# kcat/openal-soft

Measured on NVIDIA H100. Metric: voice-samples/s mixed (HRTF, bsinc24, 1024-frame updates), higher is better.
Workload: dtype f32

## Files before the change

### openal-soft_b200/csrc/async_ptx.cuh

```cuda
#pragma once
#include <cstdint>
#include <cuda_runtime.h>

namespace b200mix {

__device__ __forceinline__ uint32_t smem_u32(const void *p)
{ return static_cast<uint32_t>(__cvta_generic_to_shared(p)); }

__device__ __forceinline__ void mbar_init(uint64_t *bar, uint32_t count)
{ asm volatile("mbarrier.init.shared::cta.b64 [%0], %1;" :: "r"(smem_u32(bar)), "r"(count) : "memory"); }
__device__ __forceinline__ void mbar_fence_init()
{ asm volatile("fence.mbarrier_init.release.cluster;" ::: "memory"); }
__device__ __forceinline__ void mbar_expect_tx(uint64_t *bar, uint32_t bytes)
{ asm volatile("mbarrier.arrive.expect_tx.shared::cta.b64 _, [%0], %1;" :: "r"(smem_u32(bar)), "r"(bytes) : "memory"); }
__device__ __forceinline__ void mbar_arrive(uint64_t *bar)
{ asm volatile("mbarrier.arrive.shared::cta.b64 _, [%0];" :: "r"(smem_u32(bar)) : "memory"); }
__device__ __forceinline__ bool mbar_try_wait(uint64_t *bar, uint32_t parity)
{
    uint32_t ok;
    asm volatile("{\n\t.reg .pred p;\n\t"
                 "mbarrier.try_wait.parity.shared::cta.b64 p, [%1], %2;\n\t"
                 "selp.u32 %0, 1, 0, p;\n\t}"
                 : "=r"(ok) : "r"(smem_u32(bar)), "r"(parity) : "memory");
    return ok != 0u;
}
__device__ __forceinline__ void mbar_wait(uint64_t *bar, uint32_t parity)
{ while(!mbar_try_wait(bar, parity)) { } }

__device__ __forceinline__ void bulk_g2s(void *dst_smem, const void *src_gmem, uint32_t bytes, uint64_t *bar)
{
    asm volatile("cp.async.bulk.shared::cluster.global.mbarrier::complete_tx::bytes [%0], [%1], %2, [%3];"
        :: "r"(smem_u32(dst_smem)), "l"(src_gmem), "r"(bytes), "r"(smem_u32(bar)) : "memory");
}
__device__ __forceinline__ void fence_proxy_async_smem()
{ asm volatile("fence.proxy.async.shared::cta;" ::: "memory"); }

__device__ __forceinline__ void griddep_wait() { asm volatile("griddepcontrol.wait;" ::: "memory"); }
__device__ __forceinline__ void griddep_launch_dependents()
{ asm volatile("griddepcontrol.launch_dependents;" ::: "memory"); }

__device__ __forceinline__ uint64_t wgmma_smem_desc(uint32_t saddr, uint32_t lbo_bytes, uint32_t sbo_bytes)
{
    return uint64_t((saddr >> 4) & 0x3fffu) | (uint64_t((lbo_bytes >> 4) & 0x3fffu) << 16)
        | (uint64_t((sbo_bytes >> 4) & 0x3fffu) << 32);
}
__device__ __forceinline__ void wgmma_fence() { asm volatile("wgmma.fence.sync.aligned;" ::: "memory"); }
__device__ __forceinline__ void wgmma_commit() { asm volatile("wgmma.commit_group.sync.aligned;" ::: "memory"); }
template<int N> __device__ __forceinline__ void wgmma_wait()
{ asm volatile("wgmma.wait_group.sync.aligned %0;" :: "n"(N) : "memory"); }
__device__ __forceinline__ void wgmma_m64n16k8_tf32(float (&d)[8], uint64_t adesc, uint64_t bdesc, bool accumulate)
{
    asm volatile("{\n\t.reg .pred p;\n\tsetp.ne.b32 p, %10, 0;\n\t"
                 "wgmma.mma_async.sync.aligned.m64n16k8.f32.tf32.tf32 "
                 "{%0,%1,%2,%3,%4,%5,%6,%7}, %8, %9, p, 1, 1;\n\t}"
        : "+f"(d[0]), "+f"(d[1]), "+f"(d[2]), "+f"(d[3]), "+f"(d[4]), "+f"(d[5]), "+f"(d[6]), "+f"(d[7])
        : "l"(adesc), "l"(bdesc), "r"(uint32_t(accumulate)) : "memory");
}

}
```

### openal-soft_b200/csrc/mixer_kernels.cuh

```cuda
#pragma once
#include <cstddef>
#include <cstdint>
#include <cuda_runtime.h>

#include "voice_structs.hpp"
#include "async_ptx.cuh"

namespace b200mix {

constexpr int kLine = 1024;
constexpr int kHrirLen = 128;
constexpr int kHist = 64;
constexpr int kEdge = 24;
constexpr int kPad = 48;
constexpr int kResBuf = kLine + 256 + kPad;
constexpr int kSrcSizeMax = kResBuf - kEdge;
constexpr int kAccumLen = kLine + kHrirLen;
constexpr float kSilence = 0.00001f;
constexpr float kEps = 1.1920929e-07f;

constexpr uint32_t kVfStatic = 1u<<2, kVfLooping = 1u<<3, kVfHrtf = 1u<<4;
constexpr uint32_t kVfFading = 1u<<8, kVfHaveBuffer = 1u<<9, kVfCoefDirty = 1u<<10;
constexpr uint32_t kUpNoBuffer = 1u<<11;
constexpr uint32_t kVfChannelMask = 0xffu<<16;
// ... 810 lines not shown
            }
        }
        if(t == 0)
            newGain[c] = early ? (cg + step*float(fadeLen)) : tg;
    }
}

__device__ __forceinline__ void store_dry_gains(float *cur, const float *newGain, uint32_t cd, int t)
{
    if(t == 0)
        for(uint32_t c = 0;c < cd;++c) cur[c] = newGain[c];
}

__device__ __forceinline__ void write_back_voice(const MixParams &P, VoiceRec &rec, uint32_t v,
    uint4 h1, uint32_t flags, uint32_t vstate, uint32_t increment, bool haveBuffer, bool isQueue,
    uint4 qh, const uint32_t *qitems, bool looping, uint32_t loopStart, uint32_t loopEnd,
    uint32_t bufFrames)
{
    uint32_t newFlags = (flags | kVfFading) & ~kVfCoefDirty;
    uint32_t newState = vstate;
    uint32_t buffersDone = 0u;
    int32_t pos = int32_t(h1.x); uint32_t frac = h1.y;
    if(vstate == 2u) newState = 0u;
    else
    {
        frac += increment*P.frames;
        const uint32_t done = frac >> 16;
        pos = add_sat(pos, int32_t(done));
        frac &= 0xffffu;
        if(haveBuffer && pos > 0 && isQueue)
        {
            uint32_t item = qh.x ? qh.y : kNoLoop;
            while(item != kNoLoop)
            {
                const uint32_t len = P.buffers[qitems[item]].frames;
                if(len > uint32_t(pos)) break;
                pos -= int32_t(len);
                ++buffersDone;
                item = (item + 1u < qh.x) ? item + 1u : qh.z;
            }
            if(item == kNoLoop) { newFlags &= ~kVfHaveBuffer; newState = 2u; }
            else if(item != qh.y) P.qhdr[v].y = item;
        }
        else if(haveBuffer && pos > 0)
        {
            if(looping)
            {
                uint32_t up = uint32_t(pos);
                if(up >= loopEnd)
                    pos = int32_t((up-loopStart)%(loopEnd-loopStart) + loopStart);
            }
            else if(uint32_t(pos) >= bufFrames)
            {
                newFlags &= ~kVfHaveBuffer;
                newState = 2u;
            }
        }
        if(!haveBuffer) newState = 2u;
        rec.pos = pos; rec.frac = frac;
    }
    rec.flags = newFlags;
    rec.state = newState;
    if(P.results)
        P.results[v] = VoiceResult{pos, frac,
            newState == 1u ? 1u : (newState == 2u ? 2u : (1u<<7)), buffersDone};
}

template<int GS, int GROUPS, int CDR>
__device__ __forceinline__ void store_partial_row(const float (&accD)[CDR][kLine/GS], unsigned char *smem,
    float *partial, int g, int t)
{
    constexpr int SPT = kLine / GS;
    const size_t row = blockIdx.x;
    __syncthreads();
    float *stage = reinterpret_cast<float*>(smem);
    float *pd = partial + row*(size_t(CDR)*kLine);
    if(GROUPS == 1)
    {
        #pragma unroll
        for(int c = 0;c < CDR;++c)
            #pragma unroll
            for(int r = 0;r < SPT;++r)
                pd[c*kLine + t + r*GS] = accD[c][r];
    }
    else
    {
        for(int gg = 0;gg < GROUPS;++gg)
        {
            if(g == gg)
            {
                #pragma unroll
                for(int c = 0;c < CDR;++c)
                    #pragma unroll
                    for(int r = 0;r < SPT;++r)
                    {
                        float *dst = stage + c*kLine + t + r*GS;
                        if(gg == 0) *dst = accD[c][r]; else *dst += accD[c][r];
                    }
            }
            __syncthreads();
        }
        for(int o = threadIdx.x;o < CDR*kLine;o += GS*GROUPS) pd[o] = stage[o];
    }
}

constexpr int kMixGS = 64, kMixGroups = 2;

template<int GS, int GROUPS, int CDR>
__global__ void __launch_bounds__(GS*GROUPS, GS*GROUPS != 128 ? 1 : (CDR == 0 ? 5 : 3))
k_mix_voices(const MixParams P)
{
    using Smem = GroupSmem<CDR>;
    static_assert(CDR == 0 || sizeof(Smem)*GROUPS >= size_t(CDR)*kLine*sizeof(float),
        "the partial row is staged in the groups' storage");
    extern __shared__ __align__(16) unsigned char smem_raw[];
    const int g = threadIdx.x / GS;
    const int t = threadIdx.x % GS;
    Smem &S = reinterpret_cast<Smem*>(smem_raw)[g];
    const int bar = 1 + g;
    constexpr int SPT = kLine / GS;

    float accD[CDR > 0 ? CDR : 1][SPT];
    #pragma unroll
    for(int c = 0;c < (CDR > 0 ? CDR : 1);++c)
        #pragma unroll
        for(int r = 0;r < SPT;++r) accD[c][r] = 0.0f;

    const uint32_t n = P.frames;
    if(t == 0) { mbar_init(&S.tmaBar, 1u); mbar_fence_init(); }
    uint32_t tmaPhase = 0u;
    group_sync(bar, GS);

    const uint32_t groups = gridDim.x*GROUPS;
    for(uint32_t oi = CDR > 0 ? blockIdx.x*GROUPS + g : claim_voice(P, S.claimed, t, bar, GS, groups);
        oi < P.num_order;
        oi = CDR > 0 ? oi + groups : claim_voice(P, S.claimed, t, bar, GS, groups))
    {
        const uint32_t v = P.order[oi];
        VoiceRec &rec = P.voices[v];
        const uint4 *hp = reinterpret_cast<const uint4*>(&rec);
        const uint4 h0 = hp[0], h1 = hp[1], h2 = hp[2], h3 = hp[3];
        const uint32_t vstate = h0.x;
        if(voice_early_out(P, rec, v, vstate, h1, t)) continue;
        const uint32_t increment = h1.z;
        const uint32_t flags = h0.y;
        const bool haveBuffer = (flags & kVfHaveBuffer) != 0;
        const BufferRec rb = P.buffers[haveBuffer ? h0.z : 0u];
        const BufferRec buf = (haveBuffer && rb.pad && P.cbplan) ? P.cbplan[rb.pad - 1u] : rb;
        const uint32_t cbSlot = haveBuffer ? buf.pad : 0u;
        const uint32_t loopStart = h1.w, loopEnd = h2.x;
        int32_t intPos = int32_t(h1.x);
        uint32_t fracPos = h1.y;
        bool looping = (flags & kVfLooping) != 0 && cbSlot == 0u;
        if((flags & kVfStatic) && looping && haveBuffer && intPos >= 0
            && uint32_t(intPos) >= loopEnd)
            looping = false;
        const uint32_t resampler = h0.w;
        const bool isQueue = !(flags & kVfStatic) && P.qhdr != nullptr && cbSlot == 0u;
        const uint4 qh = isQueue ? P.qhdr[v] : make_uint4(0u, 0u, kNoLoop, 0u);
        const uint32_t *qitems = P.queue + size_t(v)*kMaxQueue;
        const bool isHrtf = CDR == 0 && P.ir_pad != 0u && (flags & kVfHrtf);
        const bool dirty = (flags & kVfCoefDirty) != 0;
        const bool isDirect = (flags & kVfDirect) != 0;
        FilterRec *dfilt = P.filt ? P.filt + size_t(v)*P.filt_paths : nullptr;
        const bool defer = dfilt && dfilt->active;
        const bool playing = vstate == 1u;

        for(int k = t;k < kPad;k += GS) S.win[k] = rec.prev[k];
        uint32_t m, tapOff, ms;
        build_phase_table<GS>(P, S.tabF, S.tabD, resampler, increment, h2, h3, t, m, tapOff, ms);
        float *xs = CDR > 0 ? S.x : P.xscratch + size_t(v)*kLine;
        if(CDR == 0) prefetch_next_voices<GS>(P, oi, groups, t);

        for(uint32_t loaded = 0;loaded < n;)
        {
            uint32_t dstn, srcn;
            calc_buffer_size(fracPos, increment, n-loaded, dstn, srcn);
            uint32_t srcDelay = 0;
            bool silent = false;
            bool packedWin = false;
            if(dstn == 0u) { dstn = n - loaded; silent = true; }
            if(intPos < 0)
            {
                srcDelay = uint32_t(-intPos);
                if(srcDelay >= srcn) silent = true;
            }
            const bool histExact = group_sync_and(bar, GS, t >= kEdge || exact16(S.win[t]));
            if(silent)
            {
                for(uint32_t k = t;k < dstn;k += GS) xs[loaded+k] = 0.0f;
                for(uint32_t k = t;k < srcn;k += GS) S.win[kEdge+k] = 0.0f;
            }
            else
            {
                float *srcBuffer = S.win + kEdge;
                bool winInt = false;
                const bool pack = resampler >= 4u && !(increment == 65536u && fracPos == 0u) && histExact;
                if(!haveBuffer) hold_end_sample<GS>(srcBuffer, srcn, t, bar);
                else
                {
                    const uint32_t uintPos = intPos < 0 ? 0u : uint32_t(intPos);
                    const uint32_t count = srcn - srcDelay;
                    for(uint32_t k = t;k < srcDelay;k += GS) srcBuffer[k] = 0.0f;
                    winInt = stage_span_tma<GS>(S.win, &S.tmaBar, tmaPhase, buf, flags, isQueue, looping,
                            loopStart, loopEnd, uintPos, srcDelay, count, pack, packedWin, t, bar)
                        || gather_span<GS>(P, buf, flags, isQueue, qh, qitems, looping, loopStart, loopEnd,
                            uintPos, count, srcBuffer + srcDelay, t, bar);
                }
                group_sync(bar, GS);

                if(pack && winInt && !packedWin)
                {
                    pack_window16<GS>(S.win, srcn, t, bar);
                    packedWin = true;
                }
                resample_chunk<GS>(S.win, S.tabF, S.tabD, xs, loaded, dstn, increment, fracPos,
                    resampler, m, tapOff, ms, packedWin, t);
            }
            advance_chunk<GS>(S.win, rec.prev, packedWin, silent, playing, n, loaded, dstn, increment,
                fracPos, intPos, t, bar);
        }
        group_sync(bar, GS);

        const uint32_t counter = (flags & kVfFading) ? (n < 64u ? n : 64u) : 0u;
        if(P.sendinfo)
            park_voice<GS, CDR>(P, xs, v, rec.send_mask, defer, isHrtf, isDirect, playing, dirty, counter, t);
        if(dfilt && !defer) filter_clear(*dfilt, t);
        if constexpr(CDR > 0)
            if(!defer && !isDirect)
                mix_dry<GS, CDR>(accD, xs, S.newGain, P.dry_cur + size_t(v)*P.cd, P.dry_tgt + size_t(v)*P.cd,
                    P.cd, n, counter, playing, t);
        if(t == 0)
            write_back_voice(P, rec, v, h1, flags, vstate, increment, haveBuffer, isQueue, qh, qitems,
                looping, loopStart, loopEnd, buf.frames);
        group_sync(bar, GS);
        if(CDR > 0 && !defer && !isDirect) store_dry_gains(P.dry_cur + size_t(v)*P.cd, S.newGain, P.cd, t);
        group_sync(bar, GS);
    }

    if constexpr(CDR > 0) store_partial_row<GS, GROUPS, CDR>(accD, smem_raw, P.partial, g, t);
    else
    {
        __syncthreads();
        griddep_launch_dependents();
    }
}

template<int GROUPS, int CDR>
union DeferredSmem {
    struct { float x[kLine]; float newGain[32]; } group[GROUPS];
    float stage[CDR*kLine];
};

template<int GS, int GROUPS, int CDR>
__global__ void __launch_bounds__(GS*GROUPS)
k_mix_deferred(const MixParams P)
{
    extern __shared__ __align__(16) unsigned char smem_raw[];
    const int g = threadIdx.x / GS;
    const int t = threadIdx.x % GS;
    auto &S = reinterpret_cast<DeferredSmem<GROUPS, CDR>*>(smem_raw)->group[g];
    const int bar = 1 + g;
    constexpr int SPT = kLine / GS;

    float accD[CDR][SPT];
    #pragma unroll
    for(int c = 0;c < CDR;++c)
        #pragma unroll
        for(int r = 0;r < SPT;++r) accD[c][r] = 0.0f;

    const uint32_t n = P.frames;
    const uint32_t groups = gridDim.x*GROUPS;
    for(uint32_t oi = blockIdx.x*GROUPS + g;oi < P.num_order;oi += groups)
    {
        const uint32_t v = P.order[oi];
        const uint32_t info = P.sendinfo[v];
        if((info & (kSiDeferred | kSiReal)) != kSiDeferred) continue;
        const float *fl = P.dline + size_t(v)*kLine;
        for(uint32_t k = t;k < n;k += GS) S.x[k] = fl[k];
        group_sync(bar, GS);
        mix_dry<GS, CDR>(accD, S.x, S.newGain, P.dry_cur + size_t(v)*P.cd, P.dry_tgt + size_t(v)*P.cd,
            P.cd, n, (info >> 8) & 0xffu, (info & kSiPlaying) != 0, t);
        group_sync(bar, GS);
        store_dry_gains(P.dry_cur + size_t(v)*P.cd, S.newGain, P.cd, t);
    }

    store_partial_row<GS, GROUPS, CDR>(accD, smem_raw, P.partial, g, t);
}

constexpr int kFirGS = 64, kFirGroups = 2, kFirCtasPerSm = 4;

__device__ __forceinline__ uint32_t next_hrtf_voice(const MixParams &P, uint32_t oi, uint32_t stride,
    uint32_t &v, uint32_t &info)
{
    for(;oi < P.num_order;oi += stride)
    {
        v = P.order[oi];
        info = P.sendinfo[v];
        if(info & kSiHrtf) break;
    }
    return oi;
}

__device__ __forceinline__ void fir_stage_issue(const MixParams &P, FirStage &B, uint64_t *bar,
    uint32_t v, uint32_t info, uint32_t n)
{
    const uint32_t lineBytes = (n & ~3u)*4u, irBytes = P.ir_pad*8u;
    const bool dirty = (info & kSiDirty) != 0;
    const float *line = ((info & kSiDeferred) ? P.dline : P.xscratch) + size_t(v)*kLine;
    fence_proxy_async_smem();
    mbar_expect_tx(bar, kHist*4u + lineBytes + (dirty ? 2u : 1u)*irBytes);
    bulk_g2s(B.x, P.voices[v].hist, kHist*4u, bar);
    if(lineBytes) bulk_g2s(B.x + kHist, line, lineBytes, bar);
    bulk_g2s(B.coefT, P.hrtf_tgt + size_t(v)*P.ir_pad, irBytes, bar);
    if(dirty) bulk_g2s(B.coefO, P.hrtf_old + size_t(v)*P.ir_pad, irBytes, bar);
}

template<int OPT, int FP>
__global__ void __launch_bounds__(kFirGS*kFirGroups, kFirCtasPerSm)
k_hrtf_fir(const MixParams P)
{
    constexpr int GS = kFirGS, GROUPS = kFirGroups;
    using Smem = FirSmem<GS, OPT, FP>;
    extern __shared__ __align__(16) unsigned char smem_raw[];
    const int g = threadIdx.x / GS;
    const int t = threadIdx.x % GS;
    Smem &S = reinterpret_cast<Smem*>(smem_raw)[g];
    const int bar = 1 + g;
    const int t0 = OPT*t;
    const uint32_t n = P.frames;

    float2 acc[OPT];
    #pragma unroll
    for(int r = 0;r < OPT;++r) acc[r] = make_float2(0.0f, 0.0f);

    for(int i = t;i < FP;i += GS) S.lLR[i] = make_float2(0.0f, 0.0f);
    for(int i = FP + int(n) + t;i < Smem::kLLen;i += GS) S.lLR[i] = make_float2(0.0f, 0.0f);
    if(t == 0) { mbar_init(&S.bar[0], 1u); mbar_init(&S.bar[1], 1u); mbar_fence_init(); }
    group_sync(bar, GS);
    griddep_wait();

    const uint32_t stride = gridDim.x*GROUPS;
    uint32_t v = 0u, info = 0u;
    uint32_t oi = next_hrtf_voice(P, blockIdx.x*GROUPS + g, stride, v, info);
    if(t == 0 && oi < P.num_order) fir_stage_issue(P, S.st[0], &S.bar[0], v, info, n);
    uint32_t parity = 0u;
    for(int b = 0;oi < P.num_order;b ^= 1)
    {
        VoiceRec &rec = P.voices[v];
        const uint4 *hp = reinterpret_cast<const uint4*>(&rec);
        const uint4 h3 = hp[3], h4 = hp[4];

        uint32_t vN = 0u, infoN = 0u;
        const uint32_t oiN = next_hrtf_voice(P, oi + stride, stride, vN, infoN);
        if(t == 0 && oiN < P.num_order) fir_stage_issue(P, S.st[b^1], &S.bar[b^1], vN, infoN, n);

        FirStage &B = S.st[b];
        const bool playing = (info & kSiPlaying) != 0;
        const bool dirty = (info & kSiDirty) != 0;
        const uint32_t counter = (info >> 8) & 0xffu;

        const float *line = ((info & kSiDeferred) ? P.dline : P.xscratch) + size_t(v)*kLine;
        for(uint32_t k = (n & ~3u) + t;k < n;k += GS) B.x[kHist + k] = line[k];
        mbar_wait(&S.bar[b], (parity >> b) & 1u);
        parity ^= 1u << b;
        if(n & 3u) group_sync(bar, GS);

        if(playing)
            for(int k = t;k < kHist;k += GS) rec.hist[k] = B.x[n + k];
        uint32_t oD0 = h4.x, oD1 = h4.y;
        float oGain = __uint_as_float(h4.z);
        const uint32_t tD0 = h3.y, tD1 = h3.z;
        const float tgtGain = __uint_as_float(h3.w);
        if(!counter) { oD0 = tD0; oD1 = tD1; oGain = tgtGain; }
        const bool sameFilter = !counter || (!dirty && oD0 == tD0 && oD1 == tD1);
        const float targetGain = tgtGain * (playing ? 1.0f : 0.0f);
        const uint32_t fademix = counter;
        float blendNewStep = 0.0f, oldStep = 0.0f;
        bool oldOn = false, newOn = false;
        float gainA = oGain;
        if(fademix)
        {
            const float gain = targetGain;
            blendNewStep = gain / float(fademix);
            oldStep = oGain / float(fademix);
            oldOn = oGain > kSilence;
            newOn = blendNewStep*float(fademix) > kSilence;
            gainA = gain;
        }
        const uint32_t todo = n - fademix;
        const float step2 = todo ? (targetGain - gainA) / float(todo) : 0.0f;

        const float *hs = B.x;
        float2 *in = S.lLR + FP;
        for(uint32_t s = t;s < fademix;s += GS)
        {
            const float gnew = (newOn && s >= 1u) ? blendNewStep*float(s) : 0.0f;
            float l = hs[kHist - tD0 + s] * gnew;
            float r = hs[kHist - tD1 + s] * gnew;
            if(sameFilter && oldOn)
            {
                const float gold = oldStep*float(fademix - s);
                l += hs[kHist - oD0 + s] * gold;
                r += hs[kHist - oD1 + s] * gold;
            }
            in[s] = make_float2(l, r);
        }
        const float *xl = hs + kHist - tD0, *xr = hs + kHist - tD1;
        for(uint32_t s = fademix + t;s < n;s += GS)
        {
            const float gnew = gainA + step2*float(s - fademix);
            in[s] = make_float2(xl[s] * gnew, xr[s] * gnew);
        }
        const bool oldPass = !sameFilter && oldOn;
        if(oldPass)
            for(int i = t;i < Smem::kOLen;i += GS)
            {
                const int s = i - FP;
                float l = 0.0f, r = 0.0f;
                if(s >= 0 && uint32_t(s) < fademix)
                {
                    const float gold = oldStep*float(fademix - uint32_t(s));
                    l = hs[kHist - oD0 + s] * gold;
                    r = hs[kHist - oD1 + s] * gold;
                }
                S.oLR[i] = make_float2(l, r);
            }
        group_sync(bar, GS);

        const int irpad = int(P.ir_pad);
        fir_pass<OPT, FP>(acc, S.lLR, B.coefT, irpad, t0);
        if(oldPass && t0 < int(kHist) + irpad)
            fir_pass<OPT, FP>(acc, S.oLR, dirty ? B.coefO : B.coefT, irpad, t0);
        if(t == 0)
        {
            rec.old_delay0 = tD0; rec.old_delay1 = tD1;
            rec.old_gain = targetGain;
        }
        group_sync(bar, GS);
        oi = oiN; v = vN; info = infoN;
    }

    const size_t row = blockIdx.x;
    __syncthreads();
    griddep_launch_dependents();
    float *stage = reinterpret_cast<float*>(smem_raw);
    for(int gg = 0;gg < GROUPS;++gg)
    {
        if(g == gg)
        {
            #pragma unroll
            for(int r = 0;r < OPT;++r)
            {
                const int o = t0 + r;
                if(o < kAccumLen)
                {
                    if(gg == 0) { stage[o] = acc[r].x; stage[kAccumLen + o] = acc[r].y; }
                    else { stage[o] += acc[r].x; stage[kAccumLen + o] += acc[r].y; }
                }
            }
            if(gg == 0 && GS*OPT < kAccumLen)
                for(int o = GS*OPT + t;o < kAccumLen;o += GS) { stage[o] = 0.0f; stage[kAccumLen + o] = 0.0f; }
        }
        __syncthreads();
    }
    float *pl = P.partial + row*(2*kAccumLen);
    for(int o = threadIdx.x;o < 2*kAccumLen;o += GS*GROUPS) pl[o] = stage[o];
}


constexpr int kReduceCols = 8, kReduceSegs = 128;

__device__ __forceinline__ float4 reduce_rows_cta(const float *__restrict__ partial, uint32_t rows,
    uint32_t len, uint32_t e4, bool live, float4 (&sm)[kReduceSegs][kReduceCols])
{
    const uint32_t col = threadIdx.x & (kReduceCols-1), seg = threadIdx.x / kReduceCols;
    float4 s = make_float4(0.f, 0.f, 0.f, 0.f);
    if(live)
    {
        const uint32_t per = (rows + kReduceSegs - 1u)/kReduceSegs;
        const uint32_t r0 = seg*per, r1 = (r0 + per < rows) ? r0 + per : rows;
        const float4 *p = reinterpret_cast<const float4*>(partial) + e4;
        const size_t stride4 = len/4u;
        constexpr uint32_t kBatch = 8;
        for(uint32_t r = r0;r < r1;r += kBatch)
        {
            float4 a[kBatch];
            #pragma unroll
            for(uint32_t k = 0;k < kBatch;++k)
                if(r + k < r1) a[k] = __ldg(p + size_t(r + k)*stride4);
            #pragma unroll
            for(uint32_t k = 0;k < kBatch;++k)
                if(r + k < r1) { s.x += a[k].x; s.y += a[k].y; s.z += a[k].z; s.w += a[k].w; }
        }
    }
    sm[seg][col] = s;
    __syncthreads();
    #pragma unroll
    for(uint32_t width = kReduceSegs/4u;width >= 1u;width /= 4u)
    {
        float4 tot = make_float4(0.f, 0.f, 0.f, 0.f);
        const bool on = seg < width;
        if(on)
        {
            tot = sm[seg*4u][col];
            #pragma unroll
            for(uint32_t k = 1;k < 4u;++k)
            {
                const float4 a = sm[seg*4u + k][col];
                tot.x += a.x; tot.y += a.y; tot.z += a.z; tot.w += a.w;
            }
        }
        __syncthreads();
        if(on) sm[seg][col] = tot;
        __syncthreads();
        if(width == 2u) break;
    }
    float4 tot = make_float4(0.f, 0.f, 0.f, 0.f);
    if(seg == 0)
    {
        tot = sm[0][col];
        const float4 b = sm[1][col];
        tot.x += b.x; tot.y += b.y; tot.z += b.z; tot.w += b.w;
    }
    return tot;
}

__global__ void __launch_bounds__(1024)
k_reduce_rows(const float *__restrict__ partial, uint32_t rows, uint32_t len,
    float *__restrict__ out, int accumulate)
{
    __shared__ float4 sm[kReduceSegs][kReduceCols];
    const uint32_t e4 = blockIdx.x*kReduceCols + (threadIdx.x & (kReduceCols-1));
    float4 tot = reduce_rows_cta(partial, rows, len, e4, e4*4u < len, sm);
    if(threadIdx.x < kReduceCols && e4*4u < len)
    {
        float4 *o = reinterpret_cast<float4*>(out) + e4;
        if(accumulate)
        {
            const float4 a = *o;
            tot.x += a.x; tot.y += a.y; tot.z += a.z; tot.w += a.w;
        }
        *o = tot;
    }
}

__global__ void __launch_bounds__(256)
k_reduce_few(const float *__restrict__ partial, uint32_t rows, uint32_t len,
    float *__restrict__ out, int accumulate)
{
    const uint32_t e4 = blockIdx.x*blockDim.x + threadIdx.x;
    if(e4*4u >= len) return;
    const float4 *p = reinterpret_cast<const float4*>(partial) + e4;
    const size_t stride4 = len/4u;
    float4 v[16];
    #pragma unroll
    for(uint32_t r = 0;r < 16u;++r)
        v[r] = r < rows ? __ldg(p + size_t(r)*stride4) : make_float4(0.f, 0.f, 0.f, 0.f);
    float4 g[4];
    #pragma unroll
    for(uint32_t j = 0;j < 4u;++j)
    {
        float4 t = v[4u*j];
        #pragma unroll
        for(uint32_t k = 1;k < 4u;++k)
        { t.x += v[4u*j+k].x; t.y += v[4u*j+k].y; t.z += v[4u*j+k].z; t.w += v[4u*j+k].w; }
        g[j] = t;
    }
    float4 tot = g[0];
    #pragma unroll
    for(uint32_t j = 1;j < 4u;++j) { tot.x += g[j].x; tot.y += g[j].y; tot.z += g[j].z; tot.w += g[j].w; }
    float4 *o = reinterpret_cast<float4*>(out) + e4;
    if(accumulate)
    {
        const float4 a = *o;
        tot.x += a.x; tot.y += a.y; tot.z += a.z; tot.w += a.w;
    }
    *o = tot;
}

struct ApplyParams {
    VoiceRec *voices; const VoiceUpdate *updates;
    const float *coeffs; const float *dry; const float *send;
    float2 *hrtf_tgt; float2 *hrtf_old; float *dry_cur, *dry_tgt, *send_cur, *send_tgt;
    uint32_t ir, ir_pad, cd, cw, num_sends;
    FilterRec *filt; uint32_t filt_paths;
    const float4 *dirs;
    const float2 *st_fields;
    const uint2 *st_elevs;
    const float2 *st_coeffs;
    const uint8_t *st_delays;
    uint32_t st_num_fields, st_ir;
    uint4 *qhdr;
    const float *real; float *real_cur, *real_tgt; uint32_t creal;
};

struct HrirBlend { uint32_t idx[4]; float w[4]; float passthru; uint32_t delay[2]; };

__device__ __forceinline__ void hrir_index(uint32_t count, float v, bool elev, uint32_t &idx, float &blend)
{
    const float inv_pi = 0.318309886183790671538f;
    if(elev)
    {
        v = __fmul_rn(__fadd_rn(__fmul_rn(inv_pi, v), 0.5f), float(count-1u));
        const uint32_t i = v > 0.0f ? uint32_t(v) : 0u;
        idx = min(i, count-1u); blend = __fsub_rn(v, float(i));
    }
    else
    {
        v = __fmul_rn(__fadd_rn(__fmul_rn(inv_pi*0.5f, v), 1.0f), float(count));
        const uint32_t i = v > 0.0f ? uint32_t(v) : 0u;
        idx = i % count; blend = __fsub_rn(v, float(i));
    }
}

__device__ __forceinline__ void hrir_blend(const ApplyParams &A, const float4 dir, HrirBlend &B)
{
    const float inv_pi = 0.318309886183790671538f;
    const float elevation = dir.x, azimuth = dir.y, distance = dir.z, spread = dir.w;
    const float dirfact = __fsub_rn(1.0f, __fmul_rn(inv_pi/2.0f, spread));
    uint32_t ebase = 0, fi = 0;
    for(;fi + 1u < A.st_num_fields;++fi)
    {
        if(distance >= A.st_fields[fi].x) break;
        ebase += __float_as_uint(A.st_fields[fi].y);
    }
    const uint32_t evCount = __float_as_uint(A.st_fields[fi].y);
    uint32_t e0i; float e0b;
    hrir_index(evCount, elevation, true, e0i, e0b);
    const uint32_t e1i = min(e0i + 1u, evCount - 1u);
    const uint2 el0 = A.st_elevs[ebase + e0i], el1 = A.st_elevs[ebase + e1i];
    uint32_t a0i, a1i; float a0b, a1b;
    hrir_index(el0.x, azimuth, false, a0i, a0b);
    hrir_index(el1.x, azimuth, false, a1i, a1b);
    B.idx[0] = el0.y + a0i; B.idx[1] = el0.y + ((a0i + 1u) % el0.x);
    B.idx[2] = el1.y + a1i; B.idx[3] = el1.y + ((a1i + 1u) % el1.x);
    const float ne = __fsub_rn(1.0f, e0b);
    B.w[0] = __fmul_rn(__fmul_rn(ne, __fsub_rn(1.0f, a0b)), dirfact);
    B.w[1] = __fmul_rn(__fmul_rn(ne, a0b), dirfact);
    B.w[2] = __fmul_rn(__fmul_rn(e0b, __fsub_rn(1.0f, a1b)), dirfact);
    B.w[3] = __fmul_rn(__fmul_rn(e0b, a1b), dirfact);
    #pragma unroll
    for(int ear = 0;ear < 2;++ear)
    {
        float dsum = __fmul_rn(float(A.st_delays[B.idx[0]*2u + ear]), B.w[0]);
        dsum = __fadd_rn(dsum, __fmul_rn(float(A.st_delays[B.idx[1]*2u + ear]), B.w[1]));
        dsum = __fadd_rn(dsum, __fmul_rn(float(A.st_delays[B.idx[2]*2u + ear]), B.w[2]));
        dsum = __fadd_rn(dsum, __fmul_rn(float(A.st_delays[B.idx[3]*2u + ear]), B.w[3]));
        B.delay[ear] = uint32_t(__float2int_rn(__fmul_rn(dsum, 0.25f)));
    }
    B.passthru = __fmul_rn(0.70710678118654752440f, __fsub_rn(1.0f, dirfact));
}

__device__ __forceinline__ void filter_reset_word(FilterRec *fr, int k)
{
    uint32_t *w = reinterpret_cast<uint32_t*>(fr);
    uint32_t val = 0u;
    if(k == 0 || k == 5 || k == 10 || k == 15) val = __float_as_uint(1.0f);
    else if(k == 24 || k == 25) val = 0xffffffffu;
    w[k] = val;
}

struct QueueSet { uint32_t voice, count, loop; uint32_t items[kMaxQueue]; };
__global__ void k_set_queue(VoiceRec *voices, uint4 *qhdr, uint32_t *queue, const QueueSet Q)
{
    const uint32_t t = threadIdx.x;
    if(t < Q.count) queue[size_t(Q.voice)*kMaxQueue + t] = Q.items[t];
    if(t == 0)
    {
        qhdr[Q.voice] = make_uint4(Q.count, 0u, Q.loop, 0u);
        uint32_t fl = voices[Q.voice].flags;
        fl = Q.count ? (fl | kVfHaveBuffer) : (fl & ~kVfHaveBuffer);
        voices[Q.voice].flags = fl;
    }
}

__global__ void k_filter_init(FilterRec *filt, size_t count)
{
    const size_t i = size_t(blockIdx.x)*blockDim.x + threadIdx.x;
    if(i < count*32u) filter_reset_word(filt + (i >> 5), int(i & 31u));
}

__global__ void k_apply_filter_updates(FilterRec *filt, uint32_t paths, const FilterUpdate *upd,
    uint32_t n)
{
    const uint32_t i = blockIdx.x*blockDim.x + threadIdx.x;
    if(i >= n*2u) return;
    const FilterUpdate &u = upd[i >> 1];
    const int f = int(i & 1u);
    FilterRec &fr = filt[size_t(u.voice)*paths + u.path];
    const float *nt = f ? u.hp : u.lp;
    bool diff = false;
    #pragma unroll
    for(int k = 0;k < 5;++k)
    {
        diff |= !(fabsf(nt[k] - fr.tgt[f][k]) <= 0.015625f);
        fr.tgt[f][k] = nt[k];
    }
    const int c = fr.counter[f];
    if(!diff)
    {
        if(c <= 0)
        {
            fr.counter[f] = 0;
            #pragma unroll
            for(int k = 0;k < 5;++k) fr.cur[f][k] = nt[k];
        }
    }
    else if(c >= 0) fr.counter[f] = 8*32;
    else
    {
// ... 941 lines not shown
```

Measured before the change: 31.98 billion.

## Prefetch first voice's history and HRIR before griddepcontrol wait in HRTF FIR

Splits the FIR stage bulk-copy issue into a fixed part (voice history and target HRIR, which do not depend on the previous kernel) and a mixed part (the line and old coefficients). The fixed part for the first voice is issued before griddep_wait, so it overlaps with the tail of the prior kernel under programmatic dependent launch. If the first order slot is not an HRTF voice, the speculative transfer is drained through an extra barrier phase. It also adds an unroll pragma on the gain-ramp loop. The risk is extra parity bookkeeping and wasted bytes when the speculation misses.

```diff
diff --git a/openal-soft_b200/csrc/async_ptx.cuh b/openal-soft_b200/csrc/async_ptx.cuh
--- a/openal-soft_b200/csrc/async_ptx.cuh
+++ b/openal-soft_b200/csrc/async_ptx.cuh
@@ -13,6 +13,8 @@
 { asm volatile("fence.mbarrier_init.release.cluster;" ::: "memory"); }
 __device__ __forceinline__ void mbar_expect_tx(uint64_t *bar, uint32_t bytes)
 { asm volatile("mbarrier.arrive.expect_tx.shared::cta.b64 _, [%0], %1;" :: "r"(smem_u32(bar)), "r"(bytes) : "memory"); }
+__device__ __forceinline__ void mbar_add_tx(uint64_t *bar, uint32_t bytes)
+{ asm volatile("mbarrier.expect_tx.relaxed.cta.shared::cta.b64 [%0], %1;" :: "r"(smem_u32(bar)), "r"(bytes) : "memory"); }
 __device__ __forceinline__ void mbar_arrive(uint64_t *bar)
 { asm volatile("mbarrier.arrive.shared::cta.b64 _, [%0];" :: "r"(smem_u32(bar)) : "memory"); }
 __device__ __forceinline__ bool mbar_try_wait(uint64_t *bar, uint32_t parity)
diff --git a/openal-soft_b200/csrc/mixer_kernels.cuh b/openal-soft_b200/csrc/mixer_kernels.cuh
--- a/openal-soft_b200/csrc/mixer_kernels.cuh
+++ b/openal-soft_b200/csrc/mixer_kernels.cuh
@@ -1136,18 +1136,29 @@
     return oi;
 }
 
-__device__ __forceinline__ void fir_stage_issue(const MixParams &P, FirStage &B, uint64_t *bar,
+__device__ __forceinline__ void fir_stage_fixed(const MixParams &P, FirStage &B, uint64_t *bar, uint32_t v)
+{
+    const uint32_t irBytes = P.ir_pad*8u;
+    fence_proxy_async_smem();
+    mbar_add_tx(bar, kHist*4u + irBytes);
+    bulk_g2s(B.x, P.voices[v].hist, kHist*4u, bar);
+    bulk_g2s(B.coefT, P.hrtf_tgt + size_t(v)*P.ir_pad, irBytes, bar);
+}
+__device__ __forceinline__ void fir_stage_mixed(const MixParams &P, FirStage &B, uint64_t *bar,
     uint32_t v, uint32_t info, uint32_t n)
 {
     const uint32_t lineBytes = (n & ~3u)*4u, irBytes = P.ir_pad*8u;
     const bool dirty = (info & kSiDirty) != 0;
     const float *line = ((info & kSiDeferred) ? P.dline : P.xscratch) + size_t(v)*kLine;
-    fence_proxy_async_smem();
-    mbar_expect_tx(bar, kHist*4u + lineBytes + (dirty ? 2u : 1u)*irBytes);
-    bulk_g2s(B.x, P.voices[v].hist, kHist*4u, bar);
+    mbar_expect_tx(bar, lineBytes + (dirty ? irBytes : 0u));
     if(lineBytes) bulk_g2s(B.x + kHist, line, lineBytes, bar);
-    bulk_g2s(B.coefT, P.hrtf_tgt + size_t(v)*P.ir_pad, irBytes, bar);
     if(dirty) bulk_g2s(B.coefO, P.hrtf_old + size_t(v)*P.ir_pad, irBytes, bar);
+}
+__device__ __forceinline__ void fir_stage_issue(const MixParams &P, FirStage &B, uint64_t *bar,
+    uint32_t v, uint32_t info, uint32_t n)
+{
+    fir_stage_fixed(P, B, bar, v);
+    fir_stage_mixed(P, B, bar, v, info, n);
 }
 
 template<int OPT, int FP>
@@ -1170,15 +1181,31 @@
 
     for(int i = t;i < FP;i += GS) S.lLR[i] = make_float2(0.0f, 0.0f);
     for(int i = FP + int(n) + t;i < Smem::kLLen;i += GS) S.lLR[i] = make_float2(0.0f, 0.0f);
-    if(t == 0) { mbar_init(&S.bar[0], 1u); mbar_init(&S.bar[1], 1u); mbar_fence_init(); }
+    const uint32_t first = blockIdx.x*GROUPS + g;
+    const bool early = first < P.num_order;
+    if(t == 0)
+    {
+        mbar_init(&S.bar[0], 1u); mbar_init(&S.bar[1], 1u); mbar_fence_init();
+        if(early) fir_stage_fixed(P, S.st[0], &S.bar[0], P.order[first]);
+    }
     group_sync(bar, GS);
     griddep_wait();
 
     const uint32_t stride = gridDim.x*GROUPS;
     uint32_t v = 0u, info = 0u;
-    uint32_t oi = next_hrtf_voice(P, blockIdx.x*GROUPS + g, stride, v, info);
-    if(t == 0 && oi < P.num_order) fir_stage_issue(P, S.st[0], &S.bar[0], v, info, n);
+    uint32_t oi = next_hrtf_voice(P, first, stride, v, info);
     uint32_t parity = 0u;
+    if(early && oi == first)
+    {
+        if(t == 0) fir_stage_mixed(P, S.st[0], &S.bar[0], v, info, n);
+    }
+    else if(early)
+    {
+        if(t == 0) mbar_arrive(&S.bar[0]);
+        mbar_wait(&S.bar[0], 0u);
+        parity = 1u;
+        if(t == 0 && oi < P.num_order) fir_stage_issue(P, S.st[0], &S.bar[0], v, info, n);
+    }
     for(int b = 0;oi < P.num_order;b ^= 1)
     {
         VoiceRec &rec = P.voices[v];
@@ -1241,6 +1268,7 @@
             in[s] = make_float2(l, r);
         }
         const float *xl = hs + kHist - tD0, *xr = hs + kHist - tD1;
+        #pragma unroll 4
         for(uint32_t s = fademix + t;s < n;s += GS)
         {
             const float gnew = gainA + step2*float(s - fademix);
```

After: 32.25 billion, median of 6. No clear change (+0.8%).
